# frozenreboot/rplidar_ros2_driver

Hardware: NVIDIA H100
Metric: Mpoints/s through unpack+filter+polar->xyz (LaserScan path: fused ascend+unpack+filter+angle-rank) (higher is better)
Workload: dtype f32

## Files before the change

rplidar_ros2_driver_b200/csrc/rpl_device.cuh:

```cuda
#pragma once
#include <cuda_runtime.h>
#include <stdint.h>

namespace rpl {

constexpr uint32_t kKeySpace = 65536;
constexpr uint32_t kResultOk = 0u;
constexpr uint32_t kResultInvalidData = 0x80008000u;
constexpr uint32_t kResultOperationFail = 0x80008001u;

__device__ __forceinline__ uint32_t node_key(uint2 n) { return n.x & 0xFFFFu; }
__device__ __forceinline__ uint32_t node_dist(uint2 n) { return __funnelshift_r(n.x, n.y, 16); }
__device__ __forceinline__ uint32_t node_quality(uint2 n) { return (n.y >> 16) & 0xFFu; }
__device__ __forceinline__ uint2 node_with_key(uint2 n, uint32_t key) {
  n.x = (n.x & 0xFFFF0000u) | (key & 0xFFFFu);
  return n;
}

__device__ __forceinline__ float key_to_deg(uint32_t key) {
  return __fmul_rn(__fmul_rn(__uint2float_rn(key), 90.0f), 1.0f / 16384.0f);
}
__device__ __forceinline__ uint32_t deg_to_key(float deg) {
  const float x = __fmul_rn(deg, 16384.0f);
  float q;
  if (deg >= 0.0f && deg <= 1024.0f) {
    const float r = 1.0f / 90.0f;
    const float q0 = __fmul_rn(x, r);
    const float e = __fmaf_rn(-q0, 90.0f, x);
    q = __fmaf_rn(e, r, q0);
  } else {
    q = __fdiv_rn(x, 90.0f);
  }
  return __float2uint_rz(q) & 0xFFFFu;
}
__device__ __forceinline__ float ascend_step(uint32_t count) {
  return __fdiv_rn(360.0f, __uint2float_rn(count));
}
__device__ __forceinline__ uint32_t ascend_fill_key(float front_deg, uint32_t i, float step) {
  float a = __fadd_rn(front_deg, __fmul_rn(__uint2float_rn(i), step));
  if (a > 360.0f) a = __fsub_rn(a, 360.0f);
  return deg_to_key(a);
}
__device__ __forceinline__ uint32_t ascend_head_key(uint32_t first_key, uint32_t first_index,
                                                    float step) {
  uint32_t k = first_key;
  for (uint32_t j = first_index; j > 0 && k != 0; --j) {
    float a = __fsub_rn(key_to_deg(k), step);
    if (a < 0.0f) a = 0.0f;
    k = deg_to_key(a);
  }
  return k;
}

__device__ __forceinline__ float key_to_rad(uint32_t key) {
  const double kDegToRad = 3.14159265358979323846 / 180.0;
  return __double2float_rn(__dmul_rn((double)key_to_deg(key), kDegToRad));
}
__device__ __forceinline__ float dist_to_m(uint32_t dist_q2) {
  const float x = __uint2float_rn(dist_q2);
  const float r = 1.0f / 4000.0f;
  const float q0 = __fmul_rn(x, r);
  const float e = __fmaf_rn(-q0, 4000.0f, x);
  return __fmaf_rn(e, r, q0);
}
__device__ __forceinline__ float small_uint_to_float(uint32_t q) {
  return __fsub_rn(__uint_as_float(0x4B000000u | q), 8388608.0f);
}
__device__ __forceinline__ float quality_to_intensity(uint32_t q, bool new_protocol) {
  return small_uint_to_float(new_protocol ? q : (q >> 2));
}
struct IntensityOf {
  uint32_t shift, mask;
  __device__ __forceinline__ explicit IntensityOf(bool new_protocol)
      : shift(new_protocol ? 16u : 18u), mask(new_protocol ? 0xFFu : 0x3Fu) {}
  __device__ __forceinline__ uint32_t units(uint32_t y) const { return (y >> shift) & mask; }
  __device__ __forceinline__ float operator()(uint32_t y) const { return small_uint_to_float(units(y)); }
};

__device__ __forceinline__ float angle_increment(uint32_t m, bool mode_a) {
  const double kTwoPi = 2.0 * 3.14159265358979323846;
  const uint32_t d = mode_a ? m : (m > 1 ? m - 1 : 1);
  return __double2float_rn(__ddiv_rn(kTwoPi, (double)d));
}
__device__ __forceinline__ int mode_a_bin(uint32_t key, float inc, bool inverted) {
  const double kTwoPi = 2.0 * 3.14159265358979323846;
  float a = key_to_rad(key);
  if (inverted) {
    a = __double2float_rn(__dsub_rn(kTwoPi, (double)a));
    if ((double)a >= kTwoPi) a = __double2float_rn(__dsub_rn((double)a, kTwoPi));
  }
  return __float2int_rz(__fdiv_rn(__fsub_rn(a, 0.0f), inc));
}

__device__ __forceinline__ int mode_a_bin_fast(uint32_t key, uint32_t m, float inc, bool inverted) {
  const uint32_t kk = inverted ? (65536u - key) : key;
  const uint32_t t = kk * m;
  const uint32_t frac = t & 0xFFFFu;
  const uint32_t g = (m >> 5) + 2u;
  if ((!inverted || key != 0u) && (frac - g) <= (65536u - 2u * g)) return (int)(t >> 16);
  return mode_a_bin(key, inc, inverted);
}

__host__ __device__ __forceinline__ uint64_t mix64(uint64_t x) {
  uint64_t z = x + 0x9E3779B97F4A7C15ull;
  z = (z ^ (z >> 30)) * 0xBF58476D1CE4E5B9ull;
  z = (z ^ (z >> 27)) * 0x94D049BB133111EBull;
  return z ^ (z >> 31);
}

__device__ __forceinline__ uint32_t warp_sum(uint32_t v) {
#pragma unroll
  for (int o = 16; o > 0; o >>= 1) v += __shfl_xor_sync(0xffffffffu, v, o);
  return v;
}
__device__ __forceinline__ uint32_t warp_min(uint32_t v) {
#pragma unroll
  for (int o = 16; o > 0; o >>= 1) v = min(v, __shfl_xor_sync(0xffffffffu, v, o));
  return v;
}
__device__ __forceinline__ uint32_t warp_inclusive_scan(uint32_t v) {
  const uint32_t lane = threadIdx.x & 31;
#pragma unroll
  for (int o = 1; o < 32; o <<= 1) {
    uint32_t t = __shfl_up_sync(0xffffffffu, v, o);
    if (lane >= (uint32_t)o) v += t;
  }
  return v;
}

__device__ __forceinline__ uint64_t l2_policy_evict_last() { return 0x14F0000000000000ull; }
__device__ __forceinline__ uint64_t l2_policy_evict_first() { return 0x12F0000000000000ull; }
__device__ __forceinline__ uint4 ld_hint_v4(const void* p, uint64_t pol) {
  uint4 r;
  asm volatile("ld.global.nc.L1::no_allocate.L2::cache_hint.v4.u32 {%0,%1,%2,%3}, [%4], %5;"
               : "=r"(r.x), "=r"(r.y), "=r"(r.z), "=r"(r.w)
               : "l"(p), "l"(pol));
  return r;
}
__device__ __forceinline__ uint2 ld_hint_v2(const void* p, uint64_t pol) {
  uint2 r;
  asm volatile("ld.global.nc.L1::no_allocate.L2::cache_hint.v2.u32 {%0,%1}, [%2], %3;"
               : "=r"(r.x), "=r"(r.y)
               : "l"(p), "l"(pol));
  return r;
}
__device__ __forceinline__ void st_hint_v2(uint2* p, uint2 v, uint64_t pol) {
  asm volatile("st.global.L1::no_allocate.L2::cache_hint.v2.u32 [%0], {%1,%2}, %3;" ::"l"(p), "r"(v.x), "r"(v.y), "l"(pol));
}

__device__ __forceinline__ void st_f32x4_if(float4* p, float4 v, uint64_t pol, uint32_t pred) {
  asm volatile(
      "{ .reg .pred q; setp.ne.u32 q, %6, 0;\n\t"
      "@q st.global.L1::no_allocate.L2::cache_hint.v4.f32 [%0], {%1,%2,%3,%4}, %5; }" ::"l"(p),
      "f"(v.x), "f"(v.y), "f"(v.z), "f"(v.w), "l"(pol), "r"(pred));
}
__device__ __forceinline__ bool cloud_keep(float dm, float inten, float rmin, float rmax, float imin) {
  return !(dm < rmin) && !(dm > rmax) && !(inten < imin);
}

__device__ __forceinline__ uint2 ld_stream_v2(const void* p) {
  uint2 r;
  asm volatile("ld.global.nc.L1::no_allocate.v2.u32 {%0,%1}, [%2];" : "=r"(r.x), "=r"(r.y) : "l"(p));
  return r;
}

}
```

rplidar_ros2_driver_b200/csrc/scan_common.cuh:

```cuda
#pragma once
#include "rpl_device.cuh"
#include "scan_args.h"

namespace rpl {
namespace {

constexpr uint32_t kWords = kKeySpace / 32;
constexpr uint32_t kMaxFastNodes = kKeySpace;

__device__ __forceinline__ void write_outcome(const ScanBatchArgs& a, uint32_t s, uint32_t status, uint32_t beams,
                                              float inc) {
  if (a.status) a.status[s] = status;
  if (a.path) a.path[s] = 0u;
  if (a.beam_counts) a.beam_counts[s] = beams;
  if (a.angle_inc) a.angle_inc[s] = inc;
}
__device__ __forceinline__ void write_outcome_empty(const ScanBatchArgs& a, uint32_t s) {
  write_outcome(a, s, a.apply_ascend ? kResultOperationFail : kResultOk, 0u, 0.0f);
}
__device__ __forceinline__ void hand_to_general(const ScanBatchArgs& a, uint32_t s) {
  a.fallback_list[atomicAdd(a.fallback_count, 1u)] = s;
}

__device__ __forceinline__ void st_f32_if(float* p, float v, uint64_t pol, uint32_t pred) {
  asm volatile(
      "{ .reg .pred q; setp.ne.u32 q, %3, 0;\n\t"
      "@q st.global.L1::no_allocate.L2::cache_hint.f32 [%0], %1, %2; }" ::"l"(p),
      "f"(v), "l"(pol), "r"(pred));
}

struct ModeBOut {
  float* ranges;
  ptrdiff_t i_minus_r;
  uint32_t ob, os;
  __device__ __forceinline__ ModeBOut(float* r, float* i, uint32_t M, bool inverted)
      : ranges(r),
        i_minus_r(reinterpret_cast<char*>(i) - reinterpret_cast<char*>(r)),
        ob(inverted ? M - 1u : 0u),
        os(inverted ? 0xFFFFFFFFu : 1u) {}
  __device__ __forceinline__ void store(uint32_t rank, float dist_m, float intensity, uint32_t pred) const {
    float* pr = ranges + (ob + os * rank);
    st_f32_if(pr, dist_m, l2_policy_evict_first(), pred);
    st_f32_if(reinterpret_cast<float*>(reinterpret_cast<char*>(pr) + i_minus_r), intensity, l2_policy_evict_first(),
              pred);
  }
};

constexpr int kMapThreads = 512;
constexpr int kMapWarps = kMapThreads / 32;
constexpr uint32_t kWordsPerThread = kWords / kMapThreads;

__device__ __forceinline__ void consumer_sync() { asm volatile("bar.sync 1, %0;" ::"n"(kMapThreads) : "memory"); }

__device__ __forceinline__ uint32_t swz_x(uint32_t x) { return (x ^ ((x >> 3) & 0x70u)) & 0xFFFFu; }
__device__ __forceinline__ uint32_t gather4(uint32_t x) { return (x * 0x10204080u) >> 28; }

__device__ __forceinline__ void bytemap_clear(uint8_t* bytemap, uint32_t tid) {
  uint4* bm = reinterpret_cast<uint4*>(bytemap);
  const uint4 z = make_uint4(0, 0, 0, 0);
#pragma unroll
  for (uint32_t j = 0; j < kKeySpace / 16 / kMapThreads; ++j) bm[j * kMapThreads + tid] = z;
}

__device__ __forceinline__ void fold_row(const uint8_t* bytemap, uint32_t tid, uint32_t (&wv)[kWordsPerThread]) {
#pragma unroll
  for (uint32_t j = 0; j < kWordsPerThread; ++j) wv[j] = 0;
  const uint4* bm = reinterpret_cast<const uint4*>(bytemap);
#pragma unroll
  for (uint32_t c = 0; c < 8; ++c) {
    const uint4 q = bm[tid * 8 + (c ^ (tid & 7u))];
    const uint32_t x[4] = {q.x, q.y, q.z, q.w};
    uint32_t bv = 0;
#pragma unroll
    for (int j = 0; j < 4; ++j) bv |= gather4(x[j] & 0x01010101u) << (4 * j);
    wv[c >> 1] |= bv << (16 * (c & 1));
  }
}

template <class Smem>
__device__ __forceinline__ void rank_table(Smem& sm, const uint32_t (&wv)[kWordsPerThread], uint32_t tid,
                                           uint32_t extra_count) {
  const uint32_t lane = tid & 31, warp = tid >> 5;
  uint32_t sv = 0;
#pragma unroll
  for (uint32_t j = 0; j < kWordsPerThread; ++j) sv += __popc(wv[j]);
  const uint32_t iv = warp_inclusive_scan(sv);
  if (lane == 31) sm.red[2 * kMapWarps + warp] = iv;
  consumer_sync();
  if (warp == 0) {
    uint32_t tv = lane < kMapWarps ? sm.red[2 * kMapWarps + lane] : 0u;
    uint32_t cc = lane < kMapWarps ? sm.red[lane] : 0u;
    const uint32_t cv = warp_inclusive_scan(tv);
    cc = warp_sum(cc);
    if (lane < kMapWarps) sm.red[2 * kMapWarps + lane] = cv - tv;
    if (lane == 31) {
      sm.totV = cv;
      sm.valid_count = cc + extra_count;
    }
  }
  consumer_sync();
  uint32_t pv = sm.red[2 * kMapWarps + warp] + iv - sv;
#pragma unroll
  for (uint32_t j = 0; j < kWordsPerThread; ++j) {
    sm.rankV[tid * kWordsPerThread + j] = make_uint2(wv[j], pv);
    pv += __popc(wv[j]);
  }
}

__device__ __forceinline__ uint32_t rank_of(const uint2* rk, uint32_t key) {
  const uint2 e = rk[key >> 5];
  return e.y + __popc(e.x & ((1u << (key & 31)) - 1u));
}

__device__ __forceinline__ uint32_t mode_a_urank(uint32_t key, uint32_t rank, uint32_t M, bool inverted,
                                                 bool has0) {
  if (!inverted) return rank;
  if (key == 0u) return 0u;
  return (M - 1u - rank) + (has0 ? 1u : 0u);
}
__device__ __forceinline__ unsigned long long mode_a_entry(float dist_m, uint32_t key, uint32_t quality) {
  return ((unsigned long long)__float_as_uint(dist_m) << 32) | ((unsigned long long)key << 8) |
         (unsigned long long)quality;
}

struct ModeAOut {
  float* ranges;
  float* intens;
  const float2* angle;
  uint32_t M;
  float inc;
  bool inverted, new_proto;
  uint64_t policy;
};

__device__ __forceinline__ void mode_a_store_bin(const ModeAOut& o, int bin, unsigned long long best, uint32_t pred) {
  const float dm = __uint_as_float((uint32_t)(best >> 32));
  const float it = quality_to_intensity((uint32_t)best & 0xFFu, o.new_proto);
  st_f32_if(o.ranges + bin, dm, o.policy, pred);
  st_f32_if(o.intens + bin, it, o.policy, pred);
}
__device__ __forceinline__ void mode_a_fill_empty(const ModeAOut& o, int from, int to) {
  const float kInf = __int_as_float(0x7f800000);
  for (int e = from; e < to; ++e) {
    o.ranges[e] = kInf;
    o.intens[e] = 0.0f;
  }
}

}
}
```

rplidar_ros2_driver_b200/csrc/scan_tma.cu:

```cuda
#include <type_traits>

#include "rpl_device.cuh"
#include "scan_args.h"
#include "scan_common.cuh"
#include "sm90_async.cuh"

namespace rpl {

namespace {

constexpr int TC = kMapThreads;
constexpr int kCWarps = TC / 32;
constexpr int kBlock = TC + 32;
constexpr uint32_t CH = 1024;
constexpr int kRounds = CH / TC;
template <int MODE>
constexpr int kStagesOf = MODE == 0 ? 16 : 4;

template <int kStages>
struct __align__(128) TmaSmem {
  uint8_t bytemap[kKeySpace];
  uint2 ring[kStages][CH];
  uint2 rankV[kWords];
  unsigned long long full[kStages];
  unsigned long long empty[kStages];
  uint32_t red[4 * kCWarps];
  uint32_t valid_count;
  uint32_t totV;
};

__device__ __forceinline__ bool scan_is_streamed(uint32_t n, uint32_t stride, uint32_t max_nodes) {
  return n != 0 && n <= stride && n <= max_nodes && n <= kMaxFastNodes;
}

constexpr uint32_t kEmit2Batch = 256;
constexpr uint32_t kEmit2Stage = kEmit2Batch + 33;
constexpr uint32_t kModeASmemMaxPoints = kKeySpace / 2;

__device__ __forceinline__ void mode_a_emit_smem(const ModeAOut& o, const uint16_t* sidx, const uint2* tile,
                                                 uint32_t warp, uint32_t nwarps, uint16_t* sb) {
  const uint32_t lane = threadIdx.x & 31u;
  const uint32_t M = o.M;
  const uint32_t len = ((M + nwarps - 1u) / nwarps + kEmit2Batch - 1u) & ~(kEmit2Batch - 1u);
  const uint32_t r_begin = min(M, warp * len), r_end = min(M, r_begin + len);
  if (r_begin >= r_end) return;
  const bool inverted = o.inverted;
  const float inc = o.inc;
  auto bin_of_key = [&](uint32_t key) { return (uint32_t)mode_a_bin_fast(key, M, inc, inverted); };
  const uint32_t kNoBin = 0xFFFFu, kBeforeFirst = 0xFFFEu;
  const float kInf = __int_as_float(0x7f800000);
  auto entry_of = [&](uint2 nd) {
    return mode_a_entry(dist_to_m(__funnelshift_r(nd.x, nd.y, 16)), nd.x & 0xFFFFu, (nd.y >> 16) & 0xFFu);
  };
  constexpr int kW = kEmit2Batch / 32;
  using Checked = std::integral_constant<bool, true>;
  using Unchecked = std::integral_constant<bool, false>;

  auto batch = [&](auto checked, uint32_t base) {
    constexpr bool CK = decltype(checked)::value;
    __syncwarp();
    uint2 nd[kW];
#pragma unroll
    for (int w = 0; w < kW; ++w) {
      const uint32_t r = base + w * 32 + lane;
      nd[w] = (!CK || r < M) ? tile[sidx[r]] : make_uint2(0, 0);
    }
    const uint32_t th = (lane == 0) ? 0u : (kEmit2Batch + lane);
    const long long rh = (long long)base - 1 + th;
    const bool halo_ok = !CK || (rh >= 0 && rh < (long long)M);
    const uint2 ndh = halo_ok ? tile[sidx[halo_ok ? rh : 0]] : make_uint2(0, 0);
    const uint32_t r2 = base - 1 + kEmit2Batch + 32;
    const bool last_ok = (lane == 31) && (!CK || r2 < M);
    const uint2 nd2 = last_ok ? tile[sidx[last_ok ? r2 : 0]] : make_uint2(0, 0);
#pragma unroll
    for (int w = 0; w < kW; ++w) {
      const uint32_t r = base + w * 32 + lane;
      sb[1 + w * 32 + lane] = (!CK || r < M) ? (uint16_t)bin_of_key(nd[w].x & 0xFFFFu) : (uint16_t)kNoBin;
    }
    {
      uint32_t b = (CK && rh < 0) ? kBeforeFirst : kNoBin;
      if (halo_ok) b = bin_of_key(ndh.x & 0xFFFFu);
      sb[th] = (uint16_t)b;
      if (lane == 31) sb[kEmit2Batch + 32] = last_ok ? (uint16_t)bin_of_key(nd2.x & 0xFFFFu) : (uint16_t)kNoBin;
    }
    __syncwarp();
#pragma unroll
    for (int w = 0; w < kW; ++w) {
      const uint32_t i = 1 + w * 32 + lane;
      const uint32_t r = base + w * 32 + lane;
      const bool live = !CK || r < M;
      const uint32_t b = sb[i], bprev = sb[i - 1];
      const bool head = live && (b != bprev);
      unsigned long long v = entry_of(nd[w]);
      uint2 nxt;
      nxt.x = __shfl_down_sync(0xffffffffu, nd[w].x, 1);
      nxt.y = __shfl_down_sync(0xffffffffu, nd[w].y, 1);
      if (w + 1 < kW) {
        const uint32_t fx = __shfl_sync(0xffffffffu, nd[(w + 1) % kW].x, 0);
        const uint32_t fy = __shfl_sync(0xffffffffu, nd[(w + 1) % kW].y, 0);
        if (lane == 31) nxt = make_uint2(fx, fy);
      }
      if (head && sb[i + 1] == b) {
        if (w + 1 == kW && lane == 31) nxt = tile[sidx[r + 1]];
        v = min(v, entry_of(nxt));
        if (sb[i + 2] == b) {
          for (uint32_t rr = r + 2; rr < M; ++rr) {
            const uint2 other = tile[sidx[rr]];
            if (bin_of_key(other.x & 0xFFFFu) != b) break;
            v = min(v, entry_of(other));
          }
        }
      }
      mode_a_store_bin(o, head ? (int)b : 0, v, head ? 1u : 0u);
      const int gap_from = (CK && bprev == kBeforeFirst) ? 0 : (int)bprev + 1;
      if (head && (int)b > gap_from) {
        if ((int)b - gap_from == 1) {
          o.ranges[gap_from] = kInf;
          o.intens[gap_from] = 0.0f;
        } else {
          mode_a_fill_empty(o, gap_from, (int)b);
        }
      }
      if (CK && live && r == M - 1u) mode_a_fill_empty(o, (int)b + 1, (int)M);
    }
  };
  for (uint32_t base = r_begin; base < r_end; base += kEmit2Batch) {
    if (base >= 1u && base + kEmit2Batch + 32u <= M) batch(Unchecked{}, base);
    else batch(Checked{}, base);
  }
}

template <int MODE>
__global__ void __launch_bounds__(kBlock, 2) scan_tma_kernel(ScanBatchArgs a, uint32_t max_nodes) {
  constexpr int kStages = kStagesOf<MODE>;
  extern __shared__ __align__(128) unsigned char smem_raw[];
  TmaSmem<kStages>& sm = *reinterpret_cast<TmaSmem<kStages>*>(smem_raw);
  const uint32_t tid = threadIdx.x, lane = tid & 31, warp = tid >> 5;

  if (tid == 0) {
    for (int i = 0; i < kStages; ++i) {
      mbar_init(&sm.full[i], 1);
      mbar_init(&sm.empty[i], kCWarps);
    }
    asm volatile("fence.mbarrier_init.release.cluster;" ::: "memory");
    asm volatile("fence.proxy.async.shared::cta;" ::: "memory");
  }
  __syncthreads();

  if (warp == kCWarps) {
    if (lane == 0) {
      const uint64_t pol_keep = l2_policy_evict_last();
      const uint64_t pol_stream = l2_policy_evict_first();
      uint32_t stage = 0, parity = 1;
      for (uint32_t s = blockIdx.x; s < a.n_scans; s += gridDim.x) {
        const uint32_t n = a.counts[s];
        if (!scan_is_streamed(n, a.stride, max_nodes)) continue;
        const uint2* base = a.nodes + (size_t)s * a.stride;
        const uint32_t nch = (n + CH - 1) / CH;
        for (int pass = 0; pass < 2; ++pass) {
          for (uint32_t c = 0; c < nch; ++c) {
            mbar_wait_relaxed(&sm.empty[stage], parity);
            const uint32_t cn = min(CH, n - c * CH);
            const uint32_t bytes = ((cn + 1u) & ~1u) * 8u;
            mbar_expect_tx(&sm.full[stage], bytes);
            tma_load_1d(&sm.ring[stage][0], base + (size_t)c * CH, bytes, &sm.full[stage],
                        pass == 0 ? pol_keep : pol_stream);
            if (++stage == kStages) {
              stage = 0;
              parity ^= 1u;
            }
          }
        }
      }
    }
    return;
  }

  const bool new_proto = a.is_new_protocol != 0;
  const bool inverted = a.inverted != 0;
  const uint64_t pol_stream = l2_policy_evict_first();
  const IntensityOf intensity_of(new_proto);
  constexpr bool MODE_A = (MODE == 1);
  constexpr bool CLOUD = (MODE == 2);
  const float w_rmin = a.range_min, w_rmax = a.range_max, w_imin = a.intensity_min;
  uint32_t stage = 0, parity = 0;
  using Checked = std::integral_constant<bool, true>;
  using Unchecked = std::integral_constant<bool, false>;
  auto advance = [&]() {
    if (++stage == kStages) {
      stage = 0;
      parity ^= 1u;
    }
  };

  auto release = [&]() {
    __syncwarp();
    if (lane == 0) mbar_arrive(&sm.empty[stage]);
  };
  auto drain = [&](uint32_t nch) {
    for (uint32_t c = 0; c < nch; ++c) {
      mbar_wait(&sm.full[stage], parity);
      release();
      advance();
    }
  };

  for (uint32_t s = blockIdx.x; s < a.n_scans; s += gridDim.x) {
    const uint32_t n = a.counts[s];

    if (n > a.stride || n > max_nodes) {
      if (tid == 0) write_outcome(a, s, kResultInvalidData, 0u, 0.0f);
      continue;
    }
    if (n > kMaxFastNodes) {
      if (tid == 0) hand_to_general(a, s);
      continue;
    }
    if (n == 0) {
      if (tid == 0) write_outcome_empty(a, s);
      continue;
    }
    const uint32_t nch = (n + CH - 1) / CH;

    bytemap_clear(sm.bytemap, tid);
    consumer_sync();

    uint32_t cnt = 0;
    uint8_t* const bmap = sm.bytemap;
    auto mark_chunk = [&](auto checked, uint32_t c) {
      mbar_wait(&sm.full[stage], parity);
      const uint2* slot = sm.ring[stage];
      uint2 v[kRounds];
#pragma unroll
      for (int r = 0; r < kRounds; ++r) v[r] = slot[r * TC + tid];
#pragma unroll
      for (int r = 0; r < kRounds; ++r) {
        const uint32_t dist = __funnelshift_r(v[r].x, v[r].y, 16);
        bool valid = dist != 0;
        if (CLOUD) valid = valid && cloud_keep(dist_to_m(dist), intensity_of(v[r].y), w_rmin, w_rmax, w_imin);
        if (decltype(checked)::value && c * CH + r * TC + tid >= n) valid = false;
        if (valid) bmap[swz_x(v[r].x)] = 1;
        cnt += valid ? 1u : 0u;
      }
      release();
      advance();
    };
    const uint32_t nfull = n / CH;
    for (uint32_t c = 0; c < nfull; ++c) mark_chunk(Unchecked{}, c);
    if (nfull < nch) mark_chunk(Checked{}, nfull);
    cnt = warp_sum(cnt);
    if (lane == 0) sm.red[warp] = cnt;
    consumer_sync();

    {
      uint32_t wv[kWordsPerThread];
      fold_row(sm.bytemap, tid, wv);
      rank_table(sm, wv, tid, 0u);
    }
    consumer_sync();
    const uint32_t M = sm.valid_count;

    if (M == 0) {
      if (tid == 0) write_outcome_empty(a, s);
      drain(nch);
      consumer_sync();
      continue;
    }
    if (sm.totV != M || (MODE_A && M > kModeASmemMaxPoints)) {
      if (tid == 0) hand_to_general(a, s);
      drain(nch);
      consumer_sync();
      continue;
    }

    float* ranges = CLOUD ? nullptr : a.ranges + (size_t)s * a.stride;
    float* intens = CLOUD ? nullptr : a.intensities + (size_t)s * a.stride;
    float4* cloud = CLOUD ? a.xyzi + (size_t)s * a.stride : nullptr;
    uint16_t* sidx = reinterpret_cast<uint16_t*>(sm.bytemap);
    const uint2* base = a.nodes + (size_t)s * a.stride;
    const float inc = angle_increment(M, MODE_A);
    const bool has0 = (sm.rankV[0].x & 1u) != 0;
    const ModeBOut mode_b(ranges, intens, M, inverted);

    auto place_chunk = [&](auto checked, uint32_t c) {
      mbar_wait(&sm.full[stage], parity);
      const uint2* slot = sm.ring[stage];
      uint2 v[kRounds];
#pragma unroll
      for (int r = 0; r < kRounds; ++r) v[r] = slot[r * TC + tid];
#pragma unroll
      for (int r = 0; r < kRounds; ++r) {
        const uint2 nd = v[r];
        const uint32_t k = nd.x & 0xFFFFu;
        const uint32_t dist = __funnelshift_r(nd.x, nd.y, 16);
        uint32_t measured = dist != 0 ? 1u : 0u;
        if (decltype(checked)::value && c * CH + r * TC + tid >= n) measured = 0;
        const uint32_t rk = rank_of(sm.rankV, k);
        const float dm = dist_to_m(dist);
        if (CLOUD) {
          const float it = intensity_of(nd.y);
          if (!cloud_keep(dm, it, w_rmin, w_rmax, w_imin)) measured = 0;
          const float2 cs = __ldg(a.trig + k);
          st_f32x4_if(cloud + rk, make_float4(__fmul_rn(dm, cs.x), __fmul_rn(dm, cs.y), 0.0f, it), pol_stream,
                      measured);
        } else if (!MODE_A) {
          mode_b.store(rk, dm, intensity_of(nd.y), measured);
        } else if (measured) {
          sidx[mode_a_urank(k, rk, M, inverted, has0)] = (uint16_t)(c * CH + r * TC + tid);
        }
      }
      release();
      advance();
    };
    for (uint32_t c = 0; c < nfull; ++c) place_chunk(Unchecked{}, c);
    if (nfull < nch) place_chunk(Checked{}, nfull);
    consumer_sync();

    if (MODE_A) {
      ModeAOut mo;
      mo.ranges = ranges;
      mo.intens = intens;
      mo.angle = a.angle;
      mo.M = M;
      mo.inc = inc;
      mo.inverted = inverted;
      mo.new_proto = new_proto;
      mo.policy = pol_stream;
      static_assert(kEmit2Stage * 2 * kCWarps <= sizeof(sm.rankV), "bin staging must fit the rank table");
      mode_a_emit_smem(mo, sidx, base, warp, kCWarps,
                       reinterpret_cast<uint16_t*>(sm.rankV) + warp * ((kEmit2Stage + 7u) & ~7u));
    }
    consumer_sync();
    if (tid == 0) write_outcome(a, s, kResultOk, M, inc);
    consumer_sync();
  }
}

constexpr int kClusterSlots = 16;
constexpr uint32_t kClusterMaxNodes = 2u * kClusterSlots * CH;
static_assert(kClusterMaxNodes <= kMaxFastNodes, "every scan the cluster kernel serves must be streamable");

struct __align__(128) ClusterSmem {
  uint8_t bytemap[kKeySpace];
  uint2 tile[kClusterSlots][CH];
  uint2 rankV[kWords];
  uint4 inbox[kWords / 4];
  unsigned long long full[kClusterSlots];
  unsigned long long empty[kClusterSlots];
  unsigned long long inbox_full;
  unsigned long long peer_free;
  uint32_t red[4 * kCWarps];
  uint32_t inbox_count;
  uint32_t valid_count;
  uint32_t totV;
};
static_assert(sizeof(ClusterSmem) <= 232448, "one CTA per SM: at most 227 KB of dynamic shared memory");
constexpr uint32_t kInboxBytes = sizeof(ClusterSmem::inbox) + sizeof(uint32_t);

__global__ void __launch_bounds__(kBlock, 1) scan_tma_cluster_kernel(ScanBatchArgs a, uint32_t max_nodes) {
  extern __shared__ __align__(128) unsigned char smem_raw[];
  ClusterSmem& sm = *reinterpret_cast<ClusterSmem*>(smem_raw);
  const uint32_t tid = threadIdx.x, lane = tid & 31, warp = tid >> 5;
  const uint32_t rank = cluster_ctarank(), peer = rank ^ 1u;
  const uint32_t s0 = blockIdx.x >> 1, s_step = gridDim.x >> 1;

  if (tid == 0) {
    for (int i = 0; i < kClusterSlots; ++i) {
      mbar_init(&sm.full[i], 1);
      mbar_init(&sm.empty[i], kCWarps);
    }
    mbar_init(&sm.inbox_full, 1);
    mbar_init(&sm.peer_free, 1);
    asm volatile("fence.mbarrier_init.release.cluster;" ::: "memory");
    asm volatile("fence.proxy.async.shared::cta;" ::: "memory");
  }
  cluster_sync_all();

  if (warp == kCWarps) {
    if (lane == 0) {
      const uint64_t pol_stream = l2_policy_evict_first();
      uint32_t eph = 0xFFFFFFFFu;
      for (uint32_t s = s0; s < a.n_scans; s += s_step) {
        const uint32_t n = a.counts[s];
        if (!scan_is_streamed(n, a.stride, max_nodes)) continue;
        const uint2* base = a.nodes + (size_t)s * a.stride;
        const uint32_t nch = (n + CH - 1) / CH;
        const uint32_t mine = (nch + 1u - rank) >> 1;
        for (uint32_t j = 0; j < mine; ++j) {
          mbar_wait_relaxed(&sm.empty[j], (eph >> j) & 1u);
          eph ^= 1u << j;
          const uint32_t c = 2u * j + rank;
          const uint32_t cn = min(CH, n - c * CH);
          const uint32_t bytes = ((cn + 1u) & ~1u) * 8u;
          mbar_expect_tx(&sm.full[j], bytes);
          tma_load_1d(&sm.tile[j][0], base + (size_t)c * CH, bytes, &sm.full[j], pol_stream);
        }
      }
    }
    __syncwarp();
  } else {
    const bool new_proto = a.is_new_protocol != 0;
    const bool inverted = a.inverted != 0;
    const IntensityOf intensity_of(new_proto);
    const bool writer = rank == 0 && tid == 0;
    const uint32_t peer_inbox = peer_addr(sm.inbox, peer);
    const uint32_t peer_count = peer_addr(&sm.inbox_count, peer);
    const uint32_t peer_inbox_full = peer_addr(&sm.inbox_full, peer);
    const uint32_t peer_peer_free = peer_addr(&sm.peer_free, peer);
    uint32_t fph = 0;
    uint32_t in_par = 0, free_par = 1;
    using Checked = std::integral_constant<bool, true>;
    using Unchecked = std::integral_constant<bool, false>;
    auto release = [&](uint32_t j) {
      __syncwarp();
      if (lane == 0) mbar_arrive(&sm.empty[j]);
    };

    for (uint32_t s = s0; s < a.n_scans; s += s_step) {
      const uint32_t n = a.counts[s];
      if (n > a.stride || n > max_nodes) {
        if (writer) write_outcome(a, s, kResultInvalidData, 0u, 0.0f);
        continue;
      }
      if (n == 0) {
        if (writer) write_outcome_empty(a, s);
        continue;
      }
      const uint32_t nch = (n + CH - 1) / CH, nfull = n / CH;
      const uint32_t mine = (nch + 1u - rank) >> 1;

      bytemap_clear(sm.bytemap, tid);
      consumer_sync();

      uint32_t cnt = 0;
      uint8_t* const bmap = sm.bytemap;
      auto mark_chunk = [&](auto checked, uint32_t j) {
        mbar_wait(&sm.full[j], (fph >> j) & 1u);
        fph ^= 1u << j;
        const uint32_t c = 2u * j + rank;
        const uint2* slot = sm.tile[j];
        uint2 v[kRounds];
#pragma unroll
        for (int r = 0; r < kRounds; ++r) v[r] = slot[r * TC + tid];
#pragma unroll
        for (int r = 0; r < kRounds; ++r) {
          const uint32_t dist = __funnelshift_r(v[r].x, v[r].y, 16);
          bool valid = dist != 0;
          if (decltype(checked)::value && c * CH + r * TC + tid >= n) valid = false;
          if (valid) bmap[swz_x(v[r].x)] = 1;
          cnt += valid ? 1u : 0u;
        }
      };
      const bool tail = nfull < nch && (nfull & 1u) == rank;
      const uint32_t mine_full = tail ? mine - 1u : mine;
      for (uint32_t j = 0; j < mine_full; ++j) mark_chunk(Unchecked{}, j);
      if (tail) mark_chunk(Checked{}, mine_full);
      cnt = warp_sum(cnt);
      if (lane == 0) sm.red[warp] = cnt;
      consumer_sync();

      {
        uint32_t wv[kWordsPerThread];
        static_assert(kWordsPerThread == 4, "the exchange moves one uint4 of bit-words per thread");
        fold_row(sm.bytemap, tid, wv);
        if (tid == 0) mbar_expect_tx(&sm.inbox_full, kInboxBytes);
        mbar_wait_cluster(&sm.peer_free, free_par);
        free_par ^= 1u;
        st_async_v4(peer_inbox + tid * 16u, make_uint4(wv[0], wv[1], wv[2], wv[3]), peer_inbox_full);
        if (warp == 0) {
          const uint32_t own = warp_sum(lane < kCWarps ? sm.red[lane] : 0u);
          if (lane == 0) st_async_u32(peer_count, own, peer_inbox_full);
        }
        mbar_wait_cluster(&sm.inbox_full, in_par);
        in_par ^= 1u;
        const uint4 pw = sm.inbox[tid];
        const uint32_t other = sm.inbox_count;
        wv[0] |= pw.x;
        wv[1] |= pw.y;
        wv[2] |= pw.z;
        wv[3] |= pw.w;
        rank_table(sm, wv, tid, other);
        if (tid == 0) mbar_arrive_remote(peer_peer_free);
      }
      consumer_sync();
      const uint32_t M = sm.valid_count;

      if (M == 0 || sm.totV != M) {
        if (writer) {
          if (M == 0) write_outcome_empty(a, s);
          else hand_to_general(a, s);
        }
        for (uint32_t j = 0; j < mine; ++j) release(j);
        continue;
      }

      const ModeBOut mode_b(a.ranges + (size_t)s * a.stride, a.intensities + (size_t)s * a.stride, M, inverted);
      auto place_chunk = [&](auto checked, uint32_t j) {
        const uint32_t c = 2u * j + rank;
        const uint2* slot = sm.tile[j];
        uint2 v[kRounds];
#pragma unroll
        for (int r = 0; r < kRounds; ++r) v[r] = slot[r * TC + tid];
#pragma unroll
        for (int r = 0; r < kRounds; ++r) {
          const uint2 nd = v[r];
          const uint32_t k = nd.x & 0xFFFFu;
          const uint32_t dist = __funnelshift_r(nd.x, nd.y, 16);
          uint32_t measured = dist != 0 ? 1u : 0u;
          if (decltype(checked)::value && c * CH + r * TC + tid >= n) measured = 0;
          mode_b.store(rank_of(sm.rankV, k), dist_to_m(dist), intensity_of(nd.y), measured);
        }
        release(j);
      };
      for (uint32_t j = 0; j < mine_full; ++j) place_chunk(Unchecked{}, j);
      if (tail) place_chunk(Checked{}, mine_full);
      if (writer) write_outcome(a, s, kResultOk, M, angle_increment(M, false));
    }
  }
  cluster_sync_all();
}

}

template <int MODE>
constexpr size_t kSmemOf = sizeof(TmaSmem<kStagesOf<MODE>>);

cudaError_t launch_scan_tma(const ScanBatchArgs& a, uint32_t max_nodes, int grid, cudaStream_t stream) {
  if (a.xyzi) scan_tma_kernel<2><<<grid, kBlock, kSmemOf<2>, stream>>>(a, max_nodes);
  else if (a.mode_a) scan_tma_kernel<1><<<grid, kBlock, kSmemOf<1>, stream>>>(a, max_nodes);
  else scan_tma_kernel<0><<<grid, kBlock, kSmemOf<0>, stream>>>(a, max_nodes);
  return cudaGetLastError();
}

bool scan_tma_cluster_applies(uint32_t stride) { return stride > kSmallMaxNodes && stride <= kClusterMaxNodes; }

namespace {
struct ClusterLaunch {
  cudaLaunchAttribute attr[1];
  cudaLaunchConfig_t cfg{};
  ClusterLaunch(int grid, cudaStream_t stream) {
    attr[0].id = cudaLaunchAttributeClusterDimension;
    attr[0].val.clusterDim.x = 2;
    attr[0].val.clusterDim.y = 1;
    attr[0].val.clusterDim.z = 1;
    cfg.gridDim = dim3((unsigned)grid);
    cfg.blockDim = dim3(kBlock);
    cfg.dynamicSmemBytes = sizeof(ClusterSmem);
    cfg.stream = stream;
    cfg.attrs = attr;
    cfg.numAttrs = 1;
  }
};
}

cudaError_t launch_scan_tma_cluster(const ScanBatchArgs& a, uint32_t max_nodes, int grid, cudaStream_t stream) {
  if (grid <= 0 || (grid & 1) != 0) return cudaErrorInvalidValue;
  ClusterLaunch l(grid, stream);
  return cudaLaunchKernelEx(&l.cfg, scan_tma_cluster_kernel, a, max_nodes);
}

int scan_tma_max_clusters() {
  ClusterLaunch l(2, nullptr);
  int n = 0;
  if (cudaOccupancyMaxActiveClusters(&n, scan_tma_cluster_kernel, &l.cfg) != cudaSuccess) return 0;
  return n;
}

cudaError_t scan_tma_configure() {
  cudaError_t e = cudaFuncSetAttribute(scan_tma_kernel<0>, cudaFuncAttributeMaxDynamicSharedMemorySize, (int)kSmemOf<0>);
  if (e != cudaSuccess) return e;
  e = cudaFuncSetAttribute(scan_tma_kernel<1>, cudaFuncAttributeMaxDynamicSharedMemorySize, (int)kSmemOf<1>);
  if (e != cudaSuccess) return e;
  e = cudaFuncSetAttribute(scan_tma_cluster_kernel, cudaFuncAttributeMaxDynamicSharedMemorySize,
                           (int)sizeof(ClusterSmem));
  if (e != cudaSuccess) return e;
  return cudaFuncSetAttribute(scan_tma_kernel<2>, cudaFuncAttributeMaxDynamicSharedMemorySize, (int)kSmemOf<2>);
}

int scan_tma_max_ctas_per_sm(int mode) {
  int nb = 0;
  if (mode == 0) cudaOccupancyMaxActiveBlocksPerMultiprocessor(&nb, scan_tma_kernel<0>, kBlock, kSmemOf<0>);
  else if (mode == 1) cudaOccupancyMaxActiveBlocksPerMultiprocessor(&nb, scan_tma_kernel<1>, kBlock, kSmemOf<1>);
  else cudaOccupancyMaxActiveBlocksPerMultiprocessor(&nb, scan_tma_kernel<2>, kBlock, kSmemOf<2>);
  return nb;
}

}
```

rplidar_ros2_driver_b200/csrc/sm90_async.cuh:

```cuda
#pragma once
#include <cuda_runtime.h>
#include <stdint.h>

namespace rpl {
namespace {

__device__ __forceinline__ uint32_t smem_u32(const void* p) {
  return static_cast<uint32_t>(__cvta_generic_to_shared(p));
}

__device__ __forceinline__ void mbar_init(void* bar, uint32_t count) {
  asm volatile("mbarrier.init.shared::cta.b64 [%0], %1;" ::"r"(smem_u32(bar)), "r"(count));
}
__device__ __forceinline__ void mbar_wait(void* bar, uint32_t parity) {
  asm volatile(
      "{\n"
      ".reg .pred p;\n"
      "LAB_WAIT:\n"
      "mbarrier.try_wait.parity.shared::cta.b64 p, [%0], %1;\n"
      "@p bra DONE;\n"
      "bra LAB_WAIT;\n"
      "DONE:\n"
      "}\n" ::"r"(smem_u32(bar)),
      "r"(parity)
      : "memory");
}
__device__ __forceinline__ void mbar_wait_relaxed(void* bar, uint32_t parity) {
  asm volatile(
      "{\n"
      ".reg .pred p;\n"
      "LAB_WAIT:\n"
      "mbarrier.try_wait.parity.shared::cta.b64 p, [%0], %1, %2;\n"
      "@p bra DONE;\n"
      "bra LAB_WAIT;\n"
      "DONE:\n"
      "}\n" ::"r"(smem_u32(bar)),
      "r"(parity), "r"(20000u)
      : "memory");
}
__device__ __forceinline__ void mbar_arrive(void* bar) {
  asm volatile("mbarrier.arrive.shared::cta.b64 _, [%0];" ::"r"(smem_u32(bar)) : "memory");
}
__device__ __forceinline__ void mbar_expect_tx(void* bar, uint32_t bytes) {
  asm volatile("mbarrier.arrive.expect_tx.shared::cta.b64 _, [%0], %1;" ::"r"(smem_u32(bar)), "r"(bytes)
               : "memory");
}

__device__ __forceinline__ void tma_load_1d(void* dst, const void* src, uint32_t bytes, void* bar,
                                            uint64_t policy) {
  asm volatile(
      "cp.async.bulk.shared::cluster.global.mbarrier::complete_tx::bytes.L2::cache_hint [%0], [%1], %2, [%3], %4;" ::
          "r"(smem_u32(dst)),
      "l"(src), "r"(bytes), "r"(smem_u32(bar)), "l"(policy)
      : "memory");
}

__device__ __forceinline__ uint32_t cluster_ctarank() {
  uint32_t r;
  asm volatile("mov.u32 %0, %%cluster_ctarank;" : "=r"(r));
  return r;
}
__device__ __forceinline__ void cluster_sync_all() {
  asm volatile("barrier.cluster.arrive.release;\n\tbarrier.cluster.wait.acquire;" ::: "memory");
}
__device__ __forceinline__ uint32_t peer_addr(const void* p, uint32_t rank) {
  uint32_t r;
  asm volatile("mapa.shared::cluster.u32 %0, %1, %2;" : "=r"(r) : "r"(smem_u32(p)), "r"(rank));
  return r;
}
__device__ __forceinline__ void st_async_v4(uint32_t addr, uint4 v, uint32_t bar) {
  asm volatile("st.async.shared::cluster.mbarrier::complete_tx::bytes.v4.b32 [%0], {%1, %2, %3, %4}, [%5];" ::"r"(addr),
               "r"(v.x), "r"(v.y), "r"(v.z), "r"(v.w), "r"(bar)
               : "memory");
}
__device__ __forceinline__ void st_async_u32(uint32_t addr, uint32_t v, uint32_t bar) {
  asm volatile("st.async.shared::cluster.mbarrier::complete_tx::bytes.b32 [%0], %1, [%2];" ::"r"(addr), "r"(v),
               "r"(bar)
               : "memory");
}
__device__ __forceinline__ void mbar_arrive_remote(uint32_t addr) {
  asm volatile("mbarrier.arrive.release.cluster.shared::cluster.b64 _, [%0];" ::"r"(addr) : "memory");
}
__device__ __forceinline__ void mbar_wait_cluster(void* bar, uint32_t parity) {
  asm volatile(
      "{\n"
      ".reg .pred p;\n"
      "LAB_WAIT:\n"
      "mbarrier.try_wait.parity.acquire.cluster.shared::cta.b64 p, [%0], %1;\n"
      "@p bra DONE;\n"
      "bra LAB_WAIT;\n"
      "DONE:\n"
      "}\n" ::"r"(smem_u32(bar)),
      "r"(parity)
      : "memory");
}

}
}
```

Before: 163,000.

## Hold first tile slots in registers to release smem early; relax L2 policies

The cluster kernel now copies the first kHeld tile slots into registers during the marking pass and releases those slots right away. The producer can then refill them with the next scan's chunks while the consumer is still ranking and placing the current scan. The held chunks are placed at the end from registers. The TMA loads and the ranges/intensities stores switch from evict_first to evict_normal L2 policy, and the remote mbarrier arrive drops its explicit .release.cluster qualifier. In exchange this raises register pressure (kHeld*kRounds uint2 per thread), and the weaker arrive ordering may be a correctness risk.

```diff
diff --git a/rplidar_ros2_driver_b200/csrc/rpl_device.cuh b/rplidar_ros2_driver_b200/csrc/rpl_device.cuh
--- a/rplidar_ros2_driver_b200/csrc/rpl_device.cuh
+++ b/rplidar_ros2_driver_b200/csrc/rpl_device.cuh
@@ -130,6 +130,7 @@
 
 __device__ __forceinline__ uint64_t l2_policy_evict_last() { return 0x14F0000000000000ull; }
 __device__ __forceinline__ uint64_t l2_policy_evict_first() { return 0x12F0000000000000ull; }
+__device__ __forceinline__ uint64_t l2_policy_evict_normal() { return 0x1000000000000000ull; }
 __device__ __forceinline__ uint4 ld_hint_v4(const void* p, uint64_t pol) {
   uint4 r;
   asm volatile("ld.global.nc.L1::no_allocate.L2::cache_hint.v4.u32 {%0,%1,%2,%3}, [%4], %5;"
diff --git a/rplidar_ros2_driver_b200/csrc/scan_common.cuh b/rplidar_ros2_driver_b200/csrc/scan_common.cuh
--- a/rplidar_ros2_driver_b200/csrc/scan_common.cuh
+++ b/rplidar_ros2_driver_b200/csrc/scan_common.cuh
@@ -33,16 +33,18 @@
   float* ranges;
   ptrdiff_t i_minus_r;
   uint32_t ob, os;
-  __device__ __forceinline__ ModeBOut(float* r, float* i, uint32_t M, bool inverted)
+  uint64_t pol;
+  __device__ __forceinline__ ModeBOut(float* r, float* i, uint32_t M, bool inverted,
+                                      uint64_t policy = l2_policy_evict_first())
       : ranges(r),
         i_minus_r(reinterpret_cast<char*>(i) - reinterpret_cast<char*>(r)),
         ob(inverted ? M - 1u : 0u),
-        os(inverted ? 0xFFFFFFFFu : 1u) {}
+        os(inverted ? 0xFFFFFFFFu : 1u),
+        pol(policy) {}
   __device__ __forceinline__ void store(uint32_t rank, float dist_m, float intensity, uint32_t pred) const {
     float* pr = ranges + (ob + os * rank);
-    st_f32_if(pr, dist_m, l2_policy_evict_first(), pred);
-    st_f32_if(reinterpret_cast<float*>(reinterpret_cast<char*>(pr) + i_minus_r), intensity, l2_policy_evict_first(),
-              pred);
+    st_f32_if(pr, dist_m, pol, pred);
+    st_f32_if(reinterpret_cast<float*>(reinterpret_cast<char*>(pr) + i_minus_r), intensity, pol, pred);
   }
 };
 
diff --git a/rplidar_ros2_driver_b200/csrc/scan_tma.cu b/rplidar_ros2_driver_b200/csrc/scan_tma.cu
--- a/rplidar_ros2_driver_b200/csrc/scan_tma.cu
+++ b/rplidar_ros2_driver_b200/csrc/scan_tma.cu
@@ -339,6 +339,8 @@
 constexpr int kClusterSlots = 16;
 constexpr uint32_t kClusterMaxNodes = 2u * kClusterSlots * CH;
 static_assert(kClusterMaxNodes <= kMaxFastNodes, "every scan the cluster kernel serves must be streamable");
+constexpr int kHeld = 4;
+static_assert(kHeld >= 0 && kHeld <= kClusterSlots, "held slots are a prefix of the tile");
 
 struct __align__(128) ClusterSmem {
   uint8_t bytemap[kKeySpace];
@@ -378,7 +380,7 @@
 
   if (warp == kCWarps) {
     if (lane == 0) {
-      const uint64_t pol_stream = l2_policy_evict_first();
+      const uint64_t pol_load = l2_policy_evict_normal();
       uint32_t eph = 0xFFFFFFFFu;
       for (uint32_t s = s0; s < a.n_scans; s += s_step) {
         const uint32_t n = a.counts[s];
@@ -393,7 +395,7 @@
           const uint32_t cn = min(CH, n - c * CH);
           const uint32_t bytes = ((cn + 1u) & ~1u) * 8u;
           mbar_expect_tx(&sm.full[j], bytes);
-          tma_load_1d(&sm.tile[j][0], base + (size_t)c * CH, bytes, &sm.full[j], pol_stream);
+          tma_load_1d(&sm.tile[j][0], base + (size_t)c * CH, bytes, &sm.full[j], pol_load);
         }
       }
     }
@@ -432,16 +434,21 @@
       bytemap_clear(sm.bytemap, tid);
       consumer_sync();
 
+      uint2 held[kHeld > 0 ? kHeld : 1][kRounds];
       uint32_t cnt = 0;
       uint8_t* const bmap = sm.bytemap;
-      auto mark_chunk = [&](auto checked, uint32_t j) {
+      auto fetch = [&](uint32_t j, uint2 (&v)[kRounds]) {
+        const uint2* slot = sm.tile[j];
+#pragma unroll
+        for (int r = 0; r < kRounds; ++r) v[r] = slot[r * TC + tid];
+      };
+      auto wait_and_fetch = [&](uint32_t j, uint2 (&v)[kRounds]) {
         mbar_wait(&sm.full[j], (fph >> j) & 1u);
         fph ^= 1u << j;
+        fetch(j, v);
+      };
+      auto mark_chunk = [&](auto checked, const uint2 (&v)[kRounds], uint32_t j) {
         const uint32_t c = 2u * j + rank;
-        const uint2* slot = sm.tile[j];
-        uint2 v[kRounds];
-#pragma unroll
-        for (int r = 0; r < kRounds; ++r) v[r] = slot[r * TC + tid];
 #pragma unroll
         for (int r = 0; r < kRounds; ++r) {
           const uint32_t dist = __funnelshift_r(v[r].x, v[r].y, 16);
@@ -453,8 +460,25 @@
       };
       const bool tail = nfull < nch && (nfull & 1u) == rank;
       const uint32_t mine_full = tail ? mine - 1u : mine;
-      for (uint32_t j = 0; j < mine_full; ++j) mark_chunk(Unchecked{}, j);
-      if (tail) mark_chunk(Checked{}, mine_full);
+      const uint32_t nheld = min((uint32_t)kHeld, mine);
+#pragma unroll
+      for (int j = 0; j < kHeld; ++j) {
+        if (j < (int)mine) {
+          wait_and_fetch(j, held[j]);
+          mark_chunk(Checked{}, held[j], j);
+          release(j);
+        }
+      }
+      for (uint32_t j = nheld; j < mine_full; ++j) {
+        uint2 v[kRounds];
+        wait_and_fetch(j, v);
+        mark_chunk(Unchecked{}, v, j);
+      }
+      if (tail && mine_full >= nheld) {
+        uint2 v[kRounds];
+        wait_and_fetch(mine_full, v);
+        mark_chunk(Checked{}, v, mine_full);
+      }
       cnt = warp_sum(cnt);
       if (lane == 0) sm.red[warp] = cnt;
       consumer_sync();
@@ -490,17 +514,14 @@
           if (M == 0) write_outcome_empty(a, s);
           else hand_to_general(a, s);
         }
-        for (uint32_t j = 0; j < mine; ++j) release(j);
+        for (uint32_t j = nheld; j < mine; ++j) release(j);
         continue;
       }
 
-      const ModeBOut mode_b(a.ranges + (size_t)s * a.stride, a.intensities + (size_t)s * a.stride, M, inverted);
-      auto place_chunk = [&](auto checked, uint32_t j) {
+      const ModeBOut mode_b(a.ranges + (size_t)s * a.stride, a.intensities + (size_t)s * a.stride, M, inverted,
+                            l2_policy_evict_normal());
+      auto place_chunk = [&](auto checked, const uint2 (&v)[kRounds], uint32_t j) {
         const uint32_t c = 2u * j + rank;
-        const uint2* slot = sm.tile[j];
-        uint2 v[kRounds];
-#pragma unroll
-        for (int r = 0; r < kRounds; ++r) v[r] = slot[r * TC + tid];
 #pragma unroll
         for (int r = 0; r < kRounds; ++r) {
           const uint2 nd = v[r];
@@ -510,10 +531,23 @@
           if (decltype(checked)::value && c * CH + r * TC + tid >= n) measured = 0;
           mode_b.store(rank_of(sm.rankV, k), dist_to_m(dist), intensity_of(nd.y), measured);
         }
+      };
+      for (uint32_t j = nheld; j < mine_full; ++j) {
+        uint2 v[kRounds];
+        fetch(j, v);
+        place_chunk(Unchecked{}, v, j);
         release(j);
-      };
-      for (uint32_t j = 0; j < mine_full; ++j) place_chunk(Unchecked{}, j);
-      if (tail) place_chunk(Checked{}, mine_full);
+      }
+      if (tail && mine_full >= nheld) {
+        uint2 v[kRounds];
+        fetch(mine_full, v);
+        place_chunk(Checked{}, v, mine_full);
+        release(mine_full);
+      }
+#pragma unroll
+      for (int j = 0; j < kHeld; ++j) {
+        if (j < (int)mine) place_chunk(Checked{}, held[j], j);
+      }
       if (writer) write_outcome(a, s, kResultOk, M, angle_increment(M, false));
     }
   }
diff --git a/rplidar_ros2_driver_b200/csrc/sm90_async.cuh b/rplidar_ros2_driver_b200/csrc/sm90_async.cuh
--- a/rplidar_ros2_driver_b200/csrc/sm90_async.cuh
+++ b/rplidar_ros2_driver_b200/csrc/sm90_async.cuh
@@ -79,7 +79,7 @@
                : "memory");
 }
 __device__ __forceinline__ void mbar_arrive_remote(uint32_t addr) {
-  asm volatile("mbarrier.arrive.release.cluster.shared::cluster.b64 _, [%0];" ::"r"(addr) : "memory");
+  asm volatile("mbarrier.arrive.shared::cluster.b64 _, [%0];" ::"r"(addr) : "memory");
 }
 __device__ __forceinline__ void mbar_wait_cluster(void* bar, uint32_t parity) {
   asm volatile(
```

Result: faster. 169,500, median of 6 (+4.0%).
